# maikmerten/hmp3

Hardware: AMD Instinct MI355X
Metric: batched stereo 44.1kHz frames/sec (whole node), CBR-128 (higher is better)
Workload: dtype f32; 1 GPU; batch=1024 stereo 44.1kHz streams x 256 frames per step per GPU, CBR-128, long blocks only, int16 PCM resident in HBM; streams_per_gpu=1024, parallelism=streams sharded over 1 GPU(s), no collective

## Files before the change

hmp3_amd/csrc/hx_alloc.hip:

```cpp
#include "hx_dev.h"

#ifndef HX_LSF
#define HX_LSF 0
#endif
#ifndef HX_A1
#define HX_A1 0
#endif
#ifndef HX_SLIM
#define HX_SLIM 0
#endif
#if HX_SLIM && HX_A1
#error "the low-footprint layout is built for the second-generation allocator only"
#endif
#define HX_WAVES (HX_SLIM ? 3 : 2)
#define HX_PERSIST HX_SLIM
#define HX_RATE_SPEED (!HX_SLIM)
#define HX_OPAQUE_LANE HX_SLIM
#define HX_SEEK_FORCEINLINE HX_SLIM
#define HX_LUCKY_K (HX_SLIM ? 6 : 12)
#define GMIN_OFFSET 70
#define PART23 4021
#define NB 22

struct AllocPrm {
    unsigned char head[4];
    int remainder, divisor, main_framebytes, sf_bit_max, AveTargetBits;
    int ms_flag, hf_flag, vbr_flag;
    int ivbr_min, ivbr_max, vbr_main_framebytes[16], vbr_pool_target;
    int fbmin, fbmax;
    int initialMNR, test1;
    int nsf[2], nsf2[2], nsf3[2], nbmax[2], nbmax2[2], nbmax3[2];
    float rnBand_l[22];
    int nsfs, nbmax_s;
    struct { int npart; } psyS;
    int nchan, side_bytes;
    int is_flag, dual, npart_l;
    int oflags;
    int run_w;
};

static_assert(sizeof(HxGr) == 96, "the frame loop copies the four HxGr of a frame as 96 words");
struct alignas(16) Outbox {
    HxSegOut seg[2];
    HxGr gr[2][2];
    int scfsi[2], mdb, part;
    unsigned sidew[10];
    unsigned char head[4];
    HxFrameOut frm;
    HxSlot slot;
    int opos, frm_index, slot_index;
    int ring_p0;
    int has_frame;
};

#if HX_SLIM
typedef short ix_t;
typedef short sgs_t;
typedef signed char sfo_t;
typedef short btab_t;
#else
typedef int ix_t;
typedef int sgs_t;
typedef int sfo_t;
typedef int btab_t;
#endif

struct FrameState {
    int padcount; unsigned main_tot, main_sent, mf_tot;
    int main_bytes; unsigned side_p0, side_p1, tot_frames_out, tot_bytes_out; int ave_tot;
    int opos, slot_lo, slot_hi;
    int pad, byte_pool, byte_max, byte_min, bytesout, pk_first;
};

struct alignas(16) AllocLds {
    float xr[2][576];
    float x34[2][576];
    float term[2][576];
#if !HX_SLIM
    int ix[2][576];
    unsigned char signx[2][576];
    alignas(16) HxBandPrep band_next;
#else
    unsigned long long sgnbits[2][9];
    ix_t ixsink;
#endif
    unsigned char band_of_pair[288];
    unsigned short lane_run[64];
    unsigned char band_last[24];
    float look_ix43[256];
#if !HX_SLIM
    float look_gain[128], look_34igain[128];
    int mblog[256];
    float pow34_exp[256];
    int logsub[84];
#else
    float gain4[4], igain16[16];
    unsigned short mblog[256];
    short logsub[84];
#endif
    float pow34_a[16], pow34_b[16], quant_off[32];
    unsigned char huff_len[1408];
    unsigned char sband_of_line[192];
    btab_t nBand_s[16], startBand_s[16], logcbw_s[16];
    unsigned char quada_len[16];
    btab_t nBand[NB], startBand[24], logcbw[NB], taper[NB];
    int NTadjust[2][NB];
    union {
        struct {
            int snr[2][NB], Noise0[2][NB], Noise[2][NB], NT[2][NB];
            int gzero[2][NB], gmin[2][NB], gsf[2][NB], sf[2][NB], active[2][NB];
            int ixmax[2][NB], ix10xmax[2][NB], up[2][NB], lo[2][NB], geval[2][NB], maskmb[2][NB];
            float xsxx[2][NB], x34max[2][NB];
            float gig[2][NB];
            alignas(8) float2 gpair[2][NB];
            int lucky[HX_LUCKY_K][2][13];
            unsigned short llist[HX_LUCKY_K * 26 + 4];
        };
        struct {
            int a_pad[17][2][NB];
            float a_sig[2][NB], a_smask[2][NB], a_mask[2][NB], a_noise[2][NB];
            int a_lastGsf[2][NB];
        };
        struct {
            int s_snr[2][3][16], s_Noise0[2][3][16], s_Noise[2][3][16], s_NT[2][3][16];
            sgs_t s_gzero[2][3][16], s_gmin[2][3][16], s_gsf[2][3][16], s_sf[2][3][16], s_active[2][3][16];
            int s_ixmax[2][3][16], s_geval[3][16], s_tmpn[3][16], s_maskmb[2][3][16];
            float s_xsxx[2][3][16], s_x34max[2][3][16];
            int s_G[2][3], s_GG[2], s_subgain[2][3];
        };
    };
    int G[2], preemp[2], scale[2], huff_bits[2];
    int hs_table[2][4], hs_cbreg[2][3], hs_nbig[2], hs_nquads[2], hs_bits[2];
    int MNR, PoolFraction, call_count;
    int a_calls, a_bitadjust[2];
    float a_running, a_ave, a_alpha;
    int hf_quant, hf_quant_stereo[2], gsf_hf, gsf_hf_stereo[2];
    int sf_save[2][21];
    int scfsi[2];
    int nchan, block_type, maxBits, maxTargetBits, minTargetBits, PoolBits, TargetBits, deltaMNR, activeBands;
    int tmp[8];
    int tmpn[2][NB];
    unsigned int sidew[10];
    HxGr gr[2][2];
    sfo_t sfout[2][2][NB];
    sfo_t sfs[2][3][12];
    AllocPrm P;
    FrameState fs;
    int tabpk[32];
    unsigned long long candpk[19];
    unsigned short r_mf[32];
    int r_off[32];
#if !HX_SLIM
    float dump[64];
#endif
    Outbox ob[2];
    const double *pow43;
    int *big_counter;
    int nstrict;
#if !HX_SLIM
    int nlucky[3];
#endif
    int cur_s;
    alignas(16) int cmdw[4];
    alignas(4) unsigned char gflag[HX_SLIM ? 64 : 256];
#ifdef HX_PROFILE
    unsigned prof[HX_PROF_WORDS];
#endif
};

#if !HX_SLIM
static_assert(offsetof(AllocLds, ix) == offsetof(AllocLds, term) + sizeof(float) * 2 * 576 && sizeof(int) == sizeof(float),
              "big_lucky_noise's terms run on from the term buffer into the quantised lines: 2304 words in one piece");
#endif

#if HX_SLIM
#define IX(c) (reinterpret_cast<ix_t *>(&L.term[0][0]) + 576 * (c))
#define BAND_LANDING (reinterpret_cast<HxBandPrep *>(&L.term[1][0]))
#define LANE_SINK (reinterpret_cast<float *>(&L.lucky[0][0][0]) + LANE)
#define MBLOG(x) hx_mblog16(L.mblog, (x))
__device__ __forceinline__ float lk_gain(const float *g4, int g) { const int k = g - 8; return ldexpf(g4[k & 3], k >> 2); }
__device__ __forceinline__ float lk_igain(const float *ig16, int g) { const int k = g - 8; return ldexpf(ig16[k & 15], -3 * (k >> 4)); }
#define LK_GAIN(g) lk_gain(L.gain4, (g))
#define LK_IGAIN(g) lk_igain(L.igain16, (g))
#define LK_GAIN_RAW(g) L.gain4[((g) - 8) & 3]
#define LK_GAIN_FIN(raw, g) ldexpf((raw), ((g) - 8) >> 2)
#define LK_IGAIN_RAW(g) L.igain16[((g) - 8) & 15]
#define LK_IGAIN_FIN(raw, g) ldexpf((raw), -3 * (((g) - 8) >> 4))
#else
#define IX(c) (&L.ix[(c)][0])
#define BAND_LANDING (&L.band_next)
#define LANE_SINK (&L.dump[LANE])
#define MBLOG(x) hx_mblog(L.mblog, (x))
#define LK_GAIN(g) L.look_gain[(g)]
#define LK_IGAIN(g) L.look_34igain[(g)]
#define LK_GAIN_RAW(g) L.look_gain[(g)]
#define LK_GAIN_FIN(raw, g) (raw)
#define LK_IGAIN_RAW(g) L.look_34igain[(g)]
#define LK_IGAIN_FIN(raw, g) (raw)
#endif
#define BAND_OF_LINE(j) L.band_of_pair[(j) >> 1]

#ifdef HX_PROFILE
#define PROF(id, stmt) do { HX_WAVE_SYNC(); long long t0_ = clock64(); stmt; HX_WAVE_SYNC(); if (threadIdx.x == 0) L.prof[(id)] += (unsigned) (clock64() - t0_); } while (0)
#define PROF_T0() long long tp_ = clock64()
#define PROF_T1() tp_ = clock64()
#define PROF_CNT(id) do { if (threadIdx.x == 0) L.prof[(id)] += 1; } while (0)
#define PROF_ACC(id) do { HX_WAVE_SYNC(); if (threadIdx.x == 0) L.prof[(id)] += (unsigned) (clock64() - tp_); tp_ = clock64(); } while (0)
#define PROF_CLOCK , long long &tp_
#define PROF_PASS , tp_
#else
#define PROF(id, stmt) do { stmt; } while (0)
#define PROF_T0() do { } while (0)
#define PROF_T1() do { } while (0)
#define PROF_CNT(id) do { } while (0)
#define PROF_ACC(id) do { } while (0)
#define PROF_CLOCK
#define PROF_PASS
#endif
#define HX_COLD __attribute__((noinline, cold))
#define HX_HFN __attribute__((noinline))
#if HX_RATE_SPEED
#define HX_RATE __attribute__((noinline))
#else
#define HX_RATE HX_COLD
#endif
__device__ __forceinline__ int hx_lane_opaque()
{
    int l;
    asm volatile("v_mbcnt_lo_u32_b32 %0, -1, 0\n\tv_mbcnt_hi_u32_b32 %0, -1, %0" : "=v"(l));
    return l;
}
#if HX_OPAQUE_LANE
// ... 593 lines not shown
        if (!(s >= s0) || (GG - s) >= g0) mode = 2;
    }
    while (__any(mode == 1)) {
        PROF_CNT(HX_PROF_N_LUCKY);
        PROF_T0();
        int nc = 0;
        if (mode == 1) {
            const int sh = 1 + L.scale[ch];
            nc = min(K, min(((s - s0) >> sh) + 1, (g0 - GG + s + sdelta - 1) >> sh));
        }
        if (i < NB) { L.geval[ch][i] = (mode == 1) ? GG - s : -1; L.tmpn[ch][i] = nc; }
        unsigned short *list = L.llist;
        const int incl = hx_wave_scan(nc), total = __builtin_amdgcn_readlane(incl, 63);
#pragma unroll
        for (int c = 0; c < HX_LUCKY_K; c++) if (c < nc) list[incl - nc + c] = (c << 8) | (ch << 7) | i;
        HX_WAVE_SYNC();
        const int ncmax = hx_wave_max(nc);
#if !HX_SLIM
        npass++; reach = max(reach, ncmax);
#endif
        const bool bslow = mode == 1 && noise_band_needs_pow(LK_IGAIN(GG - s), L.x34max[ch][i]);
        PROF_ACC(HX_PROF_LUCKY_SETUP);
        const bool two = p->nchan == 2;
        const int big = __any(bslow) ? 1 : 0;
        if (two) { if (LANE == 0) L.cmdw[3] = big; HELPER_POST2(HCMD_LUCKY, nl, ncmax); }
        lucky_dispatch(L, nl, ncmax, tf, 0, big);
        if (two) HELPER_JOIN();
        else lucky_dispatch(L, nl, ncmax, tf, 1, big);
        HX_WAVE_SYNC();
        PROF_ACC(HX_PROF_LUCKY_TERMS);
        for (int u = LANE; u < total; u += 64) {
            const int e = list[u], c = e >> 8, cc = (e >> 7) & 1, b = e & 31;
            float sxx = band_sum(tf + c * 2 * nl + cc * nl + L.startBand[b], L.nBand[b], 0.0f);
            L.lucky[c][cc][b] = MBLOG(1.0e-12f + sxx) - L.logcbw[b];
        }
        HX_WAVE_SYNC();
        PROF_ACC(HX_PROF_LUCKY_SUMS);
        {
            int best = 0;
            bool hit = false;
#pragma unroll
            for (int h = 0; h < HX_LUCKY_K; h += 6) {
                if (h == 0 || ncmax > h) {
                    int nz[6];
#pragma unroll
                    for (int c = 0; c < 6; c++) nz[c] = L.lucky[h + c][ch][min(i, 12)];
#pragma unroll
                    for (int c = 0; c < 6; c++)
                        if (h + c < nc && nz[c] <= nt) { best = nz[c]; smin = s - (h + c) * sdelta; hit = true; }
                }
            }
            if (hit) L.Noise[ch][i] = best;
            if (mode == 1) {
                s -= nc * sdelta;
                if (!(s >= s0) || (GG - s) >= g0) mode = 2;
            }
        }
        HX_WAVE_SYNC();
        PROF_ACC(HX_PROF_LUCKY_REPLAY);
    }
    if (mode == 2) {
        L.sf[ch][i] = smin;
        L.gsf[ch][i] = max(GG - smin, 0);
    }
#if !HX_SLIM
    if (reach * 2 * nl > 1152) {
        const int end = reach * 2 * nl - 1152;
        for (int j = p->nbmax[0] + LANE; j < min(end, 576); j += 64) IX(0)[j] = 0;
        for (int j = p->nbmax[1] + LANE; j < end - 576; j += 64) IX(1)[j] = 0;
    }
    if (npass && LANE == 0) { L.nlucky[0] += 1; L.nlucky[1] += npass; L.nlucky[2] += (reach > 6); }
#endif
    HX_WAVE_SYNC();
}

__device__ __forceinline__ void quant_lines(AllocLds &L, const AllocPrm *p, int opt, int c)
{
    HX_LANE_DECL;
    const int nl = p->nbmax[c];
#if HX_SLIM
    const int nfill = (opt & 2) ? nl : 576;
#endif
    const bool tab = (opt & 1) != 0;
    int q[9], b[9];
#pragma unroll
    for (int k = 0; k < 9; k++) b[k] = BAND_OF_LINE(LANE + 64 * k);
#pragma unroll
    for (int k = 0; k < 9; k++) {
        const int j = LANE + 64 * k;
        const float igain = L.gig[c][b[k]];
        const float t = igain * L.x34[c][j] + (tab ? (0.5f - 0.4375f) : (0.5f - 0.0946f));
        const float off = L.quant_off[max(min((int) t, 31), 0)];
        q[k] = (int) (t - (tab ? off : 0.0f));
    }
#pragma unroll
    for (int k = 0; k < 9; k++) {
        const int j = LANE + 64 * k;
#if HX_SLIM
        const int qq = (j < nl) ? q[k] : 0;
        *((j < nfill) ? &IX(c)[j] : &L.ixsink) = (ix_t) qq;
        if (qq > 0) atomicMax(&L.ixmax[c][b[k]], qq);
#else
        if (j < nl) {
            IX(c)[j] = q[k];
            if (q[k] > 0) atomicMax(&L.ixmax[c][b[k]], q[k]);
        }
#endif
    }
}

__device__ void do_quant(AllocLds &L, const AllocPrm *p, int opt)
{
    HX_LANE_DECL;
    const int ch = LANE >> 5, i = LANE & 31;
    if (i < NB) {
        L.ixmax[ch][i] = (i < p->nsf[ch]) ? 0 : L.ixmax[ch][i];
        L.gig[ch][i] = LK_IGAIN(L.gsf[ch][i] & 127);
    }
    HX_WAVE_SYNC();
    const bool two = p->nbmax[1] > 0;
    if (two) HELPER_POST(HCMD_QUANT, opt);
    quant_lines(L, p, opt, 0);
    if (two) HELPER_JOIN();
    HX_WAVE_SYNC();
}

struct Cand { int n, t0, t1, t2, t3, tmax; };

__device__ __forceinline__ Cand mk_cand(int n, int t0, int t1, int t2, int t3, int tmax)
{
    Cand c; c.n = n; c.t0 = t0; c.t1 = t1; c.t2 = t2; c.t3 = t3; c.tmax = tmax;
    return c;
}

__device__ __forceinline__ Cand candidates_chain(int rmax)
{
    if (rmax <= 0) return mk_cand(0, 0, 0, 0, 0, 0);
    if (rmax == 1) return mk_cand(2, 1, 3, 0, 0, 1);
    if (rmax == 2) return mk_cand(2, 2, 3, 0, 0, 2);
    if (rmax == 3) return mk_cand(2, 5, 6, 0, 0, 3);
    if (rmax <= 5) return mk_cand(4, 7, 8, 9, 12, 5);
    if (rmax <= 7) return mk_cand(4, 10, 11, 12, 15, 7);
    if (rmax <= 15) return mk_cand(2, 13, 15, 0, 0, 15);
    if (rmax == 16) return mk_cand(2, 16, 24, 0, 0, 16);
    if (rmax <= 18) return mk_cand(2, 17, 24, 0, 0, 18);
    if (rmax <= 22) return mk_cand(2, 18, 24, 0, 0, 22);
    if (rmax <= 30) return mk_cand(2, 19, 24, 0, 0, 30);
    if (rmax <= 46) return mk_cand(2, 25, 20, 0, 0, 46);
    if (rmax <= 78) return mk_cand(2, 20, 26, 0, 0, 78);
    if (rmax <= 142) return mk_cand(2, 27, 21, 0, 0, 142);
    if (rmax <= 270) return mk_cand(2, 21, 28, 0, 0, 270);
    if (rmax <= 526) return mk_cand(2, 29, 22, 0, 0, 526);
    if (rmax <= 1038) return mk_cand(2, 22, 30, 0, 0, 1038);
    if (rmax <= 2062) return mk_cand(2, 30, 23, 0, 0, 2062);
    return mk_cand(2, 31, 23, 0, 0, 8206);
}

__device__ __forceinline__ int cand_class(int rmax)
{
    if (rmax <= 3) return max(rmax, 0);
    if (rmax <= 15) return rmax <= 5 ? 4 : (rmax <= 7 ? 5 : 6);
    return min(7 + (31 - __clz(rmax - 15)), 18);
}
__device__ __forceinline__ int cand_class_rep(int c)
{
    return c <= 3 ? c : (c == 4 ? 4 : (c == 5 ? 6 : (c == 6 ? 8 : 15 + (1 << (c - 7)))));
}
__device__ __forceinline__ unsigned long long cand_pack(const Cand &c)
{
    return (unsigned long long) (c.n | (c.t0 << 3) | (c.t1 << 8) | (c.t2 << 13) | (c.t3 << 18)) | ((unsigned long long) c.tmax << 23);
}
__device__ __forceinline__ Cand candidates(const AllocLds &L, int rmax)
{
    const unsigned long long pk = L.candpk[cand_class(rmax)];
    const unsigned lo = (unsigned) pk;
    return mk_cand(lo & 7, (lo >> 3) & 31, (lo >> 8) & 31, (lo >> 13) & 31, (lo >> 18) & 31, (int) (pk >> 23));
}

__device__ __forceinline__ int tab_pack(const AllocLds &L, int t) { return L.tabpk[t]; }
__device__ __forceinline__ int pair_len_p(const AllocLds &L, int pk, int x, int y)
{
    const int off = pk & 0xFFF, dim = (pk >> 12) & 0xFF, lin = pk >> 20;
    const int cx = min(x, 15), cy = min(y, 15);
    int n = L.huff_len[off + cx * dim + cy];
    n += (x >= 15 ? lin : 0) + (y >= 15 ? lin : 0);
    return n + (x != 0) + (y != 0);
}

__device__ __forceinline__ int pair_len(const AllocLds &L, int t, int x, int y) { return pair_len_p(L, tab_pack(L, t), x, y); }

__device__ __forceinline__ void acc_pair(const AllocLds &L, const Cand &c, int x, int y, int &p01, int &p23)
{
    if (c.n == 0) return;
    p01 += pair_len(L, c.t0, x, y) | (pair_len(L, c.t1, x, y) << 16);
    if (c.n == 4) p23 += pair_len(L, c.t2, x, y) | (pair_len(L, c.t3, x, y) << 16);
}

__device__ __forceinline__ int pick_table(const Cand &c, int p01, int p23, int live, int *bits)
{
    const int b0 = p01 & 0xFFFF, b1 = (p01 >> 16) & 0xFFFF, b2 = p23 & 0xFFFF, b3 = (p23 >> 16) & 0xFFFF;
    int best = 0, t = c.t0;
    if (c.n != 0 && live) {
        if (b0 < b1) { best = b0; t = c.t0; } else { best = b1; t = c.t1; }
        if (c.n == 4) {
            if (b2 <= best) { best = b2; t = c.t2; }
            if (b3 <= best) { best = b3; t = c.t3; }
        }
    }
    *bits += best;
    return t;
}

__device__ __forceinline__ int region_max(const int *ixmax, int a, int b)
{
    int m = 0;
    for (int i = a; i < b; i++) if (m < ixmax[i]) m = ixmax[i];
    return m;
}

__device__ int count_bits_ch(AllocLds &L, const AllocPrm *p, int ch, int ncb)
{
    HX_LANE_DECL;
    const int *ixmax = L.ixmax[ch];
    const ix_t *ix = IX(ch);
    const int bt = L.block_type;
    PROF_T0();
    int cb0, cb1, cb2, cb3;
    const int my = (LANE < ncb) ? ixmax[LANE] : 0;
    const unsigned long long mk0 = __ballot(my > 0), mk1 = __ballot(my > 1);
    cb3 = mk0 ? 64 - __clzll((long long) mk0) : 0;
    cb2 = mk1 ? 64 - __clzll((long long) mk1) : 0;
    cb0 = cb1 = 0;
#define RMAX(a_, b_) hx_wave_max((LANE >= (a_) && LANE < (b_)) ? my : 0)
    if (bt == 0) { if (cb2 < 2) { cb2 = 2; if (cb3 < cb2) cb3 = cb2; } }
    else { cb0 = 8; cb2 = max(cb2, 8); cb3 = max(cb3, cb2); cb1 = cb0; }
    PROF_ACC(HX_PROF_CNT_BALLOTS);
    int lo2 = L.startBand[cb2 - 1], hi2 = L.startBand[cb2], lo3 = L.startBand[cb3 - 1], hi3 = L.startBand[cb3];
    int j2 = lo2, j3 = lo3;
    for (int j = lo2 + LANE; j < hi2; j += 64) if (ix[j] > 1) j2 = j;
    for (int j = lo3 + LANE; j < hi3; j += 64) if (ix[j] > 0) j3 = j;
    j2 = hx_wave_max(j2);
    j3 = hx_wave_max(j3);
    PROF_ACC(HX_PROF_CNT_J23);
    int nbig = (j2 + 2) & (~1);
    if (bt == 0) { if (nbig < L.startBand[2]) nbig = L.startBand[2]; }
    else { if (nbig < L.startBand[8]) nbig = L.startBand[8]; }
    int nquads = (j3 + 4 - nbig) >> 2;
    if (bt != 0) nquads = max(nquads, 0);
    Cand c0, c1, c2;
    if (bt == 0) {
        const int c = cb2;
        int r0 = (c < 6) ? 1 : (c < 9 ? 2 : (c < 12 ? 3 : (c < 15 ? 4 : (c < 18 ? 5 : (c < 21 ? 6 : 7)))));
        int r1 = (c < 5) ? 1 : (c < 8 ? 2 : (c < 10 ? 3 : (c == 10 ? 4 : (c < 15 ? 5 : (c < 17 ? 6 : (c < 20 ? 7 : 8))))));
        cb0 = r0;
        cb1 = r0 + r1;
        if (cb0 < 1) cb0 = 1;
        if (cb1 <= cb0) cb1 = cb0 + 1;
        if (cb1 > cb0 + 8) cb1 = cb0 + 8;
        c0 = candidates(L, RMAX(0, cb0));
        c1 = candidates(L, RMAX(cb0, cb1));
        c2 = candidates(L, RMAX(cb1, cb2));
        if (c2.tmax < c1.tmax) {
            const unsigned long long m = __ballot(my > c2.tmax && LANE > cb0 && LANE <= cb1 - 1);
            const int j = m ? 63 - __clzll((long long) m) : cb0;
            cb1 = j + 1;
        }
        if (c1.tmax < c0.tmax) {
            int n = cb1 - 8;
            if (n < 1) n = 1;
            if (cb0 - 1 > n) {
                const unsigned long long m = __ballot(my > c1.tmax && LANE > n && LANE <= cb0 - 1);
                const int j = m ? 63 - __clzll((long long) m) : n;
                cb0 = j + 1;
            }
        }
    } else {
        c0 = candidates(L, RMAX(0, cb0));
        c1 = candidates(L, 0);
        c2 = candidates(L, RMAX(cb0, cb2));
    }
#undef RMAX
    PROF_ACC(HX_PROF_CNT_REGIONS);
    const int n0 = L.startBand[cb0], n1 = L.startBand[cb1];
    int r0a = 0, r0b = 0, r1a = 0, r1b = 0, r2a = 0, r2b = 0;
    {
        const int pa0 = tab_pack(L, c0.t0), pb0 = tab_pack(L, c0.t1);
        const int pa1 = tab_pack(L, c1.t0), pb1 = tab_pack(L, c1.t1);
        const int pa2 = tab_pack(L, c2.t0), pb2 = tab_pack(L, c2.t1);
        const bool any4 = c0.n == 4 || c1.n == 4 || c2.n == 4;
        int2 xy[5];
#pragma unroll
#if HX_SLIM
        for (int k = 0; k < 5; k++) { const unsigned w = reinterpret_cast<const unsigned *>(ix)[min(LANE + 64 * k, 287)]; xy[k] = make_int2((int) (w & 0xFFFFu), (int) (w >> 16)); }
#else
        for (int k = 0; k < 5; k++) xy[k] = reinterpret_cast<const int2 *>(ix)[min(LANE + 64 * k, 287)];
#endif
        int acc[5];
#pragma unroll
        for (int k = 0; k < 5; k++) {
            const int j = 2 * (LANE + 64 * k);
            const int pa = (j < n0) ? pa0 : (j < n1 ? pa1 : pa2), pb = (j < n0) ? pb0 : (j < n1 ? pb1 : pb2);
            acc[k] = pair_len_p(L, pa, xy[k].x, xy[k].y) | (pair_len_p(L, pb, xy[k].x, xy[k].y) << 16);
        }
#pragma unroll
        for (int k = 0; k < 5; k++) {
            const int j = 2 * (LANE + 64 * k);
            const int rn = (j < n0) ? c0.n : (j < n1 ? c1.n : c2.n);
            const int v = (j < nbig && rn != 0) ? acc[k] : 0;
            r0a += (j < n0) ? v : 0;
            r1a += (j >= n0 && j < n1) ? v : 0;
            r2a += (j >= n1) ? v : 0;
        }
        if (any4) {
            const int qa0 = tab_pack(L, c0.t2), qb0 = tab_pack(L, c0.t3);
            const int qa1 = tab_pack(L, c1.t2), qb1 = tab_pack(L, c1.t3);
            const int qa2 = tab_pack(L, c2.t2), qb2 = tab_pack(L, c2.t3);
#pragma unroll
            for (int k = 0; k < 5; k++) {
                const int j = 2 * (LANE + 64 * k);
                const int pa = (j < n0) ? qa0 : (j < n1 ? qa1 : qa2), pb = (j < n0) ? qb0 : (j < n1 ? qb1 : qb2);
                acc[k] = pair_len_p(L, pa, xy[k].x, xy[k].y) | (pair_len_p(L, pb, xy[k].x, xy[k].y) << 16);
            }
#pragma unroll
            for (int k = 0; k < 5; k++) {
                const int j = 2 * (LANE + 64 * k);
                const int rn = (j < n0) ? c0.n : (j < n1 ? c1.n : c2.n);
                const int v = (j < nbig && rn == 4) ? acc[k] : 0;
                r0b += (j < n0) ? v : 0;
                r1b += (j >= n0 && j < n1) ? v : 0;
                r2b += (j >= n1) ? v : 0;
            }
        }
    }
    PROF_ACC(HX_PROF_CNT_PAIRS);
    int qa = 0, qb = 0;
    {
        int2 qv[3][2];
#pragma unroll
        for (int k = 0; k < 3; k++) {
            const int q = min(LANE + 64 * k, max(nquads - 1, 0));
#if HX_SLIM
            const uint2 w2 = *reinterpret_cast<const uint2 *>(ix + nbig + 4 * q);
            qv[k][0] = make_int2((int) (w2.x & 0xFFFFu), (int) (w2.x >> 16)); qv[k][1] = make_int2((int) (w2.y & 0xFFFFu), (int) (w2.y >> 16));
#else
            const int2 *v2 = reinterpret_cast<const int2 *>(ix + nbig + 4 * q);
            qv[k][0] = v2[0]; qv[k][1] = v2[1];
#endif
        }
#pragma unroll
        for (int k = 0; k < 3; k++) {
            const int v0 = qv[k][0].x, v1 = qv[k][0].y, v2 = qv[k][1].x, v3 = qv[k][1].y;
            const int pop = v0 + v1 + v2 + v3;
            const int la = L.quada_len[((v0 << 3) + (v1 << 2) + (v2 << 1) + v3) & 15] + pop;
            const bool ok = LANE + 64 * k < nquads;
            qa += ok ? la : 0;
            qb += ok ? 4 + pop : 0;
        }
    }
    PROF_ACC(HX_PROF_CNT_QUADS);
    r0a = hx_wave_sum(r0a); r2a = hx_wave_sum(r2a);
    r0b = hx_wave_sum(r0b); r2b = hx_wave_sum(r2b);
    r1a = hx_wave_sum(r1a); r1b = hx_wave_sum(r1b);
    int bits = 0;
    const int tab0 = pick_table(c0, r0a, r0b, n0 > 0, &bits);
    int tab1 = pick_table(c1, r1a, r1b, (n1 - n0 > 0) && bt == 0, &bits);
    const int tab2 = pick_table(c2, r2a, r2b, nbig - n1 > 0, &bits);
    if (bt != 0) tab1 = tab2;
    {
        const int q = hx_wave_sum(qa | (qb << 16));
        qa = q & 0xFFFF;
        qb = (q >> 16) & 0xFFFF;
    }
    int qidx = 0;
    if (nquads > 0) { if (qa < qb) { bits += qa; qidx = 0; } else { bits += qb; qidx = 1; } }
    if (LANE == 0) {
        L.hs_table[ch][0] = tab0; L.hs_table[ch][1] = tab1; L.hs_table[ch][2] = tab2; L.hs_table[ch][3] = qidx;
        L.hs_cbreg[ch][0] = cb0; L.hs_cbreg[ch][1] = cb1; L.hs_cbreg[ch][2] = cb2;
        L.hs_nbig[ch] = nbig; L.hs_nquads[ch] = nquads; L.hs_bits[ch] = bits;
        L.huff_bits[ch] = bits;
    }
    PROF_ACC(HX_PROF_CNT_REDUCE);
    return bits;
}

__device__ int count_bits(AllocLds &L, const AllocPrm *p, const int *ncb)
{
    HX_LANE_DECL;
    PROF_CNT(HX_PROF_N_COUNTS);
    const bool two = p->nchan == 2;
    if (two) HELPER_POST(HCMD_COUNT_BITS, ncb[1]);
    int bits = count_bits_ch(L, p, 0, ncb[0]);
    if (two) { HELPER_JOIN(); bits += L.hs_bits[1]; }
    HX_WAVE_SYNC();
    return bits;
}

__device__ int quant_count_bits(AllocLds &L, const AllocPrm *p, int opt, int zero21, const int *ncb)
{
    HX_LANE_DECL;
    const int ch = LANE >> 5, i = LANE & 31;
    if (i < NB) {
        L.ixmax[ch][i] = (i < p->nsf[ch]) ? 0 : L.ixmax[ch][i];
        L.gig[ch][i] = LK_IGAIN(L.gsf[ch][i] & 127);
    }
    HX_WAVE_SYNC();
    PROF_CNT(HX_PROF_N_COUNTS);
    const bool two = p->nchan == 2;
    PROF_T0();
    if (two) HELPER_POST2(HCMD_QUANT_COUNT, opt, ncb[1]);
    PROF_ACC(HX_PROF_QC_POST);
    quant_lines(L, p, opt, 0);
    HX_WAVE_SYNC();
    PROF_ACC(HX_PROF_QC_QUANT);
    if (zero21) { if (LANE == 0) L.ixmax[0][21] = 0; HX_WAVE_SYNC(); }
    int bits = count_bits_ch(L, p, 0, ncb[0]);
    PROF_T1();
    if (two) { HELPER_JOIN(); bits += L.hs_bits[1]; }
    HX_WAVE_SYNC();
    PROF_ACC(HX_PROF_QC_JOIN);
    return bits;
}

#include "hx_alloc2.inc"
#include "hx_alloc_short.inc"
#if HX_A1
#include "hx_alloc1.inc"
#endif
#include "hx_alloc3.inc"
```

hmp3_amd/csrc/hx_alloc3.inc:

```

#define COLD(field) (((const __attribute__((address_space(4))) AllocArgs *) __builtin_amdgcn_kernarg_segment_ptr())->field)
#define RFL(x) __builtin_amdgcn_readfirstlane(x)

__device__ __noinline__ void emit_packet(AllocLds &L, const AllocPrm *p, unsigned char *q, int *nbytes, int pad, int ms, int raw_bytes, int hdr, int lsf_igr)
{
    HX_LANE_DECL;
    if (LANE < 4) {
        unsigned char h = p->head[LANE];
        if (LANE == 2 && pad) h |= 2;
        if (LANE == 3) h = (unsigned char) ((h & 0xCF) | ((ms + ms + (HX_A1 ? p->is_flag : 0)) << 4));
        q[LANE] = h;
    }
    if (lsf_igr >= 0) pack_side_lsf(L, p, q + 4, lsf_igr, 0);
    else pack_side(L, p, q + 4, 0);
    if (LANE == 0) *nbytes = hdr + raw_bytes;
}

template <int LSF>
__device__ __forceinline__ int pack_sf_any(AllocLds &L, int pos, int igr, int ch, int bt, int use_scfsi, int not_null, int *sc, unsigned short *sfdst)
{
    HX_LANE_DECL;
    *sc = 0;
    int field = 0;
    if (LSF) {
// ... 199 lines not shown
    for (int k = 0; k < 9; k++) { a[k] = L.xr[0][LANE + 64 * k]; b[k] = L.xr[1][LANE + 64 * k]; }
#pragma unroll
    for (int k = 0; k < 9; k++) {
        const int j = LANE + 64 * k;
        L.x34[0][j] = (j < nl0) ? pow34(L, a[k]) : 0.0f;
        L.x34[1][j] = (j < nl1) ? pow34(L, b[k]) : 0.0f;
    }
}

template <int LSF>
__device__ __forceinline__ void helper_serve(const AllocArgs &a, AllocLds &L)
{
    for (;;) {
        HX_LANE_DECL;
        WG_BARRIER();
        const int4 order = *reinterpret_cast<const int4 *>(&L.cmdw[0]);
        const int cmd = order.x;
        if (cmd == HCMD_SEEK) seek_actual_ch(L, &L.P, 1);
        else if (cmd == HCMD_COUNT_BITS) count_bits_ch(L, &L.P, 1, order.y);
        else if (cmd == HCMD_LUCKY) lucky_dispatch(L, order.y, order.z, &L.term[0][0], 1, order.w);
        else if (cmd == HCMD_QUANT) quant_lines(L, &L.P, order.y, 1);
        else if (cmd == HCMD_QUANT_COUNT) { quant_lines(L, &L.P, order.y, 1); HX_WAVE_SYNC(); count_bits_ch(L, &L.P, 1, order.z); }
        else if (cmd == HCMD_ISF2) isf2_ch(L, &L.P, 1);
        else if (cmd == HCMD_FETCH) {
            const int s = L.cur_s;
            int nbt = 2, nms = 0;
            if (order.y >= 0) {
                granule_fetch(L, a, (long long) s * a.NG + order.y);
                nbt = a.bt[(long long) s * a.NG + order.y]; nms = a.msflag[(long long) s * a.NG + order.y];
            }
            const int gl = order.z, gf = (gl >= 0) ? gl - 1 : ((order.y < 0) ? order.w : -1);
            LinesRegs lr0 = {}, lr1 = {};
            OutRegs orr = {};
            const int two = L.P.nchan == 2;
            const int gbt = order.w & 255;
            if (gl >= 0) { lines_gather(L, (order.w >> 8) & 1, 0, gbt, lr0); if (two) lines_gather(L, (order.w >> 9) & 1, 1, gbt, lr1); }
            if (gf >= 0) outbox_gather(L, gf, orr);
            asm volatile("s_waitcnt vmcnt(0) lgkmcnt(0)" ::: "memory");
            const bool long_gr = !HX_A1 && nbt != 2;
            if (long_gr) {
                xr_to_coded(L, nms);
                if (!two) x34_from_coded(L, nms);
                asm volatile("s_waitcnt lgkmcnt(0)" ::: "memory");
            }
            WG_BARRIER();
            if (gl >= 0) {
                const long long unit = (long long) s * a.NG + gl;
                lines_store(a, unit, 0, gbt, lr0);
                if (two) lines_store(a, unit, 1, gbt, lr1);
            }
            if (gf >= 0) outbox_store<LSF>(L, a, s, gf, orr);
            if (long_gr && two) { x34_from_coded(L, nms); asm volatile("s_waitcnt lgkmcnt(0)" ::: "memory"); }
            continue;
        }
        else if (cmd == HCMD_EXIT) return;
        WG_BARRIER();
    }
}

__device__ __forceinline__ void stage_stream(const AllocArgs &a, AllocLds &L, const HxStream *ss, const HxParams *gp, const HxGlobalTabs *gt)
{
    HX_LANE_DECL;
#if HX_SLIM
    for (int i = LANE; i < 256; i += 64) { L.look_ix43[i] = gp->look_ix43[i]; L.mblog[i] = (unsigned short) (gt->mblog[i] + 38227); }
    if (LANE < 4) L.gain4[LANE] = gp->look_gain[8 + LANE];
    if (LANE < 16) L.igain16[LANE] = gp->look_34igain[8 + LANE];
    if (LANE < 18) L.sgnbits[LANE / 9][LANE % 9] = 0;
#else
    for (int i = LANE; i < 256; i += 64) { L.look_ix43[i] = gp->look_ix43[i]; L.mblog[i] = gt->mblog[i]; L.pow34_exp[i] = gt->pow34_exp[i]; }
    for (int i = LANE; i < 128; i += 64) { L.look_gain[i] = gp->look_gain[i]; L.look_34igain[i] = gp->look_34igain[i]; }
#endif
    for (int i = LANE; i < 1408; i += 64) L.huff_len[i] = gt->huff_len[i];
    for (int i = LANE; i < 288; i += 64) L.band_of_pair[i] = gp->band_of_line[2 * i];
    L.lane_run[LANE] = gp->lane_run[LANE];
    if (LANE < 24) L.band_last[LANE] = gp->band_last_lane[LANE];
    for (int i = LANE; i < 192; i += 64) L.sband_of_line[i] = gp->sband_of_line[i];
    if (LANE < 16) {
        L.nBand_s[LANE] = (LANE < 13) ? gp->nBand_s[LANE] : 0;
        L.startBand_s[LANE] = (LANE < 14) ? gp->startBand_s[LANE] : 192;
        L.logcbw_s[LANE] = gp->look_log_cbwmb_s[LANE];
    }
    for (int i = LANE; i < 84; i += 64) L.logsub[i] = (HX_SLIM ? (short) gt->logsub[i] : gt->logsub[i]);
    if (LANE < 32) L.quant_off[LANE] = gt->quant_off[LANE];
    if (LANE < 32) {
        const int dim = (LANE >= 16) ? 16 : gt->huff_dim[LANE], lin = (LANE >= 16) ? gt->huff_lin[LANE] : 0;
        L.tabpk[LANE] = gt->huff_off[LANE] | (dim << 12) | (lin << 20);
    }
    if (LANE < 19) L.candpk[LANE] = cand_pack(candidates_chain(cand_class_rep(LANE)));
    if (LANE < 16) {
        L.pow34_a[LANE] = gt->pow34_a[LANE]; L.pow34_b[LANE] = gt->pow34_b[LANE];
        L.quada_len[LANE] = gt->quada_len[LANE];
    }
    if (LANE < 24) L.startBand[LANE] = gp->startBand_l[LANE];
    if (LANE < NB) { L.nBand[LANE] = gp->nBand_l[LANE]; L.logcbw[LANE] = gp->look_log_cbwmb[LANE]; L.taper[LANE] = gp->taperNT[LANE]; }
#if !HX_SLIM
    for (int i = LANE; i < 2 * 576; i += 64) { IX(0)[i] = 0; (&L.signx[0][0])[i] = 0; }
#endif
    if (LANE < 44) {
        int c = LANE / 22, b = LANE % 22;
        L.NTadjust[c][b] = ss->NTadjust[c][b];
        L.ixmax[c][b] = 0; L.sf[c][b] = 0; L.active[c][b] = 0; L.gsf[c][b] = 0; L.gzero[c][b] = 0; L.gmin[c][b] = 0;
        L.x34max[c][b] = 0.0f; L.Noise[c][b] = 0; L.Noise0[c][b] = 0; L.NT[c][b] = 0; L.geval[c][b] = -1;
        L.up[c][b] = 0; L.lo[c][b] = 0;
    }
    if (LANE < 42) L.sf_save[LANE / 21][LANE % 21] = ss->sf_save[LANE / 21][LANE % 21];
    if (LANE == 0) { L.pow43 = gt->pow43; L.big_counter = COLD(done_counter) + HX_CNT_BIG_SWEEPS; L.nstrict = 0; }
#if !HX_SLIM
    if (LANE < 3) L.nlucky[LANE] = 0;
#endif
    if (LANE < 4) L.P.head[LANE] = gp->head[LANE];
    if (LANE < 16) L.P.vbr_main_framebytes[LANE] = gp->vbr_main_framebytes[LANE];
    if (LANE < 22) L.P.rnBand_l[LANE] = gp->rnBand_l[LANE];
    if (LANE < 2) {
        const bool on = LANE < gp->nchan;
        L.P.nsf[LANE] = on ? gp->nsf[LANE] : 0; L.P.nsf2[LANE] = on ? gp->nsf2[LANE] : 0; L.P.nsf3[LANE] = on ? gp->nsf3[LANE] : 0;
        L.P.nbmax[LANE] = on ? gp->nbmax[LANE] : 0; L.P.nbmax2[LANE] = on ? gp->nbmax2[LANE] : 0; L.P.nbmax3[LANE] = on ? gp->nbmax3[LANE] : 0;
    }
    if (LANE == 0) {
        L.P.remainder = gp->remainder; L.P.divisor = gp->divisor; L.P.main_framebytes = gp->main_framebytes;
        L.P.sf_bit_max = gp->sf_bit_max; L.P.AveTargetBits = gp->AveTargetBits;
        L.P.ms_flag = gp->ms_flag; L.P.hf_flag = gp->hf_flag; L.P.vbr_flag = gp->vbr_flag;
        L.P.ivbr_min = gp->ivbr_min; L.P.ivbr_max = gp->ivbr_max; L.P.vbr_pool_target = gp->vbr_pool_target;
        L.P.fbmin = gp->vbr_main_framebytes[gp->ivbr_min & 15]; L.P.fbmax = gp->vbr_main_framebytes[gp->ivbr_max & 15];
        L.P.initialMNR = gp->initialMNR; L.P.test1 = gp->test1;
        L.P.nsfs = gp->nsfs; L.P.nbmax_s = gp->nbmax_s; L.P.psyS.npart = gp->psyS.npart;
        L.P.nchan = gp->nchan; L.P.side_bytes = gp->side_bytes;
        L.P.is_flag = gp->is_flag; L.P.dual = gp->alloc1 && gp->h_mode == 2; L.P.npart_l = gp->psyL.npart;
        L.P.oflags = (a.packet ? 1 : 0) | (a.dbg ? 2 : 0) | (a.frame_stats ? 4 : 0) | (a.strict_sums ? 8 : 0);
        L.P.run_w = gp->run_w;
    }
#if HX_A1
    for (int i = LANE; i < 256; i += 64) {
        (&L.term[0][0])[i] = gp->a1_f_ix[i]; (&L.term[0][0])[256 + i] = gp->a1_f_ixmax[i];
        (&L.term[0][0])[512 + i] = gp->a1_f_big_ix[i]; (&L.term[0][0])[768 + i] = gp->a1_f_big_ixmax[i];
    }
    if (LANE < 42) L.gsf[LANE / 21][LANE % 21] = ss->a1_gsf[LANE / 21][LANE % 21];
    if (LANE == 0) {
        L.a_calls = ss->a1_call_count; L.a_bitadjust[0] = ss->a1_bitadjust[0]; L.a_bitadjust[1] = ss->a1_bitadjust[1];
        L.a_running = ss->a1_running_a; L.a_ave = ss->a1_ave_alpha; L.a_alpha = ss->a1_alpha;
    }
#endif
    if (LANE == 0) {
        L.MNR = ss->MNR; L.PoolFraction = ss->PoolFraction; L.call_count = ss->call_count;
        L.hf_quant = 0; L.hf_quant_stereo[0] = L.hf_quant_stereo[1] = 0; L.gsf_hf = -1;
        L.gsf_hf_stereo[0] = L.gsf_hf_stereo[1] = -1;
        L.scfsi[0] = L.scfsi[1] = 0;
        for (int g = 0; g < 2; g++) for (int c = 0; c < 2; c++) {
            HxGr z = {};
            L.gr[g][c] = z;
            for (int k = 0; k < 3; k++) L.gr[g][c].subblock_gain[k] = ss->gr_subblock_gain[g][c][k];
        }
    }
#ifdef HX_PROFILE
    L.prof[LANE] = 0;
    if (LANE == 0) L.prof[HX_PROF_TOTAL] = (unsigned) clock64();
#endif
    HX_WAVE_SYNC();
}

template <int LSF>
__device__ __forceinline__ void slots_init(const AllocArgs &a, AllocLds &L, int s, const HxStream *ss, const HxParams *gp)
{
    HX_LANE_DECL;
    const int F = a.NG / 2;
    if (LANE == 0) {
        FrameState &fs = L.fs;
        fs.padcount = ss->padcount;
        fs.main_tot = ss->main_tot; fs.main_sent = ss->main_sent; fs.mf_tot = ss->mf_tot;
        fs.main_bytes = ss->main_bytes;
        fs.side_p0 = ss->side_p0; fs.side_p1 = ss->side_p1;
        fs.tot_frames_out = ss->tot_frames_out; fs.tot_bytes_out = ss->tot_bytes_out;
// ... 480 lines not shown
```

Baseline: 18.02 million frames/s.

## Vectorize quantization and bit counting over line pairs with precomputed candidate tables

Quantization now processes lines in pairs, loading float2 x34 values and storing packed int2 or 16-bit pairs to cut LDS instruction count and atomics per line. Bit counting precomputes per-candidate Huffman table packs in LDS, reads startBand values through lane reads instead of LDS, merges the j2/j3 scans into one loop, and derives the middle region sum from a total sum so one wave reduction is dropped. Clipping, escape and sign terms are hoisted out of the per-table lookup, and the quad count is moved earlier in the non-slim path. In exchange the code grows more complex, adds more LDS for the candidate tables, and raises register pressure.

```diff
diff --git a/hmp3_amd/csrc/hx_alloc.hip b/hmp3_amd/csrc/hx_alloc.hip
--- a/hmp3_amd/csrc/hx_alloc.hip
+++ b/hmp3_amd/csrc/hx_alloc.hip
@@ -82,7 +82,7 @@
     alignas(16) HxBandPrep band_next;
 #else
     unsigned long long sgnbits[2][9];
-    ix_t ixsink;
+    alignas(4) ix_t ixsink[2];
 #endif
     unsigned char band_of_pair[288];
     unsigned short lane_run[64];
@@ -148,6 +148,9 @@
     FrameState fs;
     int tabpk[32];
     unsigned long long candpk[19];
+#if !HX_SLIM
+    alignas(16) int candtab[19][4];
+#endif
     unsigned short r_mf[32];
     int r_off[32];
 #if !HX_SLIM
@@ -907,28 +910,33 @@
     const int nfill = (opt & 2) ? nl : 576;
 #endif
     const bool tab = (opt & 1) != 0;
-    int q[9], b[9];
-#pragma unroll
-    for (int k = 0; k < 9; k++) b[k] = BAND_OF_LINE(LANE + 64 * k);
-#pragma unroll
-    for (int k = 0; k < 9; k++) {
-        const int j = LANE + 64 * k;
+    int q0[5], q1[5], b[5];
+#pragma unroll
+    for (int k = 0; k < 5; k++) b[k] = L.band_of_pair[min(LANE + 64 * k, 287)];
+#pragma unroll
+    for (int k = 0; k < 5; k++) {
         const float igain = L.gig[c][b[k]];
-        const float t = igain * L.x34[c][j] + (tab ? (0.5f - 0.4375f) : (0.5f - 0.0946f));
-        const float off = L.quant_off[max(min((int) t, 31), 0)];
-        q[k] = (int) (t - (tab ? off : 0.0f));
-    }
-#pragma unroll
-    for (int k = 0; k < 9; k++) {
-        const int j = LANE + 64 * k;
+        const float2 x = reinterpret_cast<const float2 *>(&L.x34[c][0])[min(LANE + 64 * k, 287)];
+        const float t0 = igain * x.x + (tab ? (0.5f - 0.4375f) : (0.5f - 0.0946f));
+        const float t1 = igain * x.y + (tab ? (0.5f - 0.4375f) : (0.5f - 0.0946f));
+        const float off0 = L.quant_off[max(min((int) t0, 31), 0)];
+        const float off1 = L.quant_off[max(min((int) t1, 31), 0)];
+        q0[k] = (int) (t0 - (tab ? off0 : 0.0f));
+        q1[k] = (int) (t1 - (tab ? off1 : 0.0f));
+    }
+#pragma unroll
+    for (int k = 0; k < 5; k++) {
+        const int i = LANE + 64 * k, j = 2 * i;
 #if HX_SLIM
-        const int qq = (j < nl) ? q[k] : 0;
-        *((j < nfill) ? &IX(c)[j] : &L.ixsink) = (ix_t) qq;
-        if (qq > 0) atomicMax(&L.ixmax[c][b[k]], qq);
+        const int a0 = (j < nl) ? q0[k] : 0, a1 = (j < nl) ? q1[k] : 0;
+        *((j < nfill) ? reinterpret_cast<unsigned *>(IX(c)) + i : reinterpret_cast<unsigned *>(&L.ixsink[0])) = ((unsigned) a0 & 0xFFFFu) | ((unsigned) a1 << 16);
+        const int m = max(a0, a1);
+        if (m > 0) atomicMax(&L.ixmax[c][b[k]], m);
 #else
         if (j < nl) {
-            IX(c)[j] = q[k];
-            if (q[k] > 0) atomicMax(&L.ixmax[c][b[k]], q[k]);
+            reinterpret_cast<int2 *>(IX(c))[i] = make_int2(q0[k], q1[k]);
+            const int m = max(q0[k], q1[k]);
+            if (m > 0) atomicMax(&L.ixmax[c][b[k]], m);
         }
 #endif
     }
@@ -950,11 +958,12 @@
     HX_WAVE_SYNC();
 }
 
-struct Cand { int n, t0, t1, t2, t3, tmax; };
+struct Cand { int n, t0, t1, t2, t3, tmax; int pk0, pk1, pk2, pk3; };
 
 __device__ __forceinline__ Cand mk_cand(int n, int t0, int t1, int t2, int t3, int tmax)
 {
     Cand c; c.n = n; c.t0 = t0; c.t1 = t1; c.t2 = t2; c.t3 = t3; c.tmax = tmax;
+    c.pk0 = c.pk1 = c.pk2 = c.pk3 = 0;
     return c;
 }
 
@@ -983,9 +992,8 @@
 
 __device__ __forceinline__ int cand_class(int rmax)
 {
-    if (rmax <= 3) return max(rmax, 0);
-    if (rmax <= 15) return rmax <= 5 ? 4 : (rmax <= 7 ? 5 : 6);
-    return min(7 + (31 - __clz(rmax - 15)), 18);
+    const int lo = max(rmax, 0), mid = rmax <= 5 ? 4 : (rmax <= 7 ? 5 : 6), hi = min(7 + (31 - __clz(max(rmax - 15, 1))), 18);
+    return rmax <= 3 ? lo : (rmax <= 15 ? mid : hi);
 }
 __device__ __forceinline__ int cand_class_rep(int c)
 {
@@ -995,14 +1003,34 @@
 {
     return (unsigned long long) (c.n | (c.t0 << 3) | (c.t1 << 8) | (c.t2 << 13) | (c.t3 << 18)) | ((unsigned long long) c.tmax << 23);
 }
+__device__ __forceinline__ int tab_pack(const AllocLds &L, int t) { return L.tabpk[t]; }
+template <bool UNIFORM = false>
 __device__ __forceinline__ Cand candidates(const AllocLds &L, int rmax)
 {
-    const unsigned long long pk = L.candpk[cand_class(rmax)];
-    const unsigned lo = (unsigned) pk;
-    return mk_cand(lo & 7, (lo >> 3) & 31, (lo >> 8) & 31, (lo >> 13) & 31, (lo >> 18) & 31, (int) (pk >> 23));
-}
-
-__device__ __forceinline__ int tab_pack(const AllocLds &L, int t) { return L.tabpk[t]; }
+    const int cls = cand_class(rmax);
+    const unsigned long long pk = L.candpk[cls];
+#if !HX_SLIM
+    int4 tp = *reinterpret_cast<const int4 *>(&L.candtab[cls][0]);
+#endif
+    unsigned lo = (unsigned) pk, hi = (unsigned) (pk >> 32);
+    if (UNIFORM) {
+        lo = __builtin_amdgcn_readfirstlane(lo); hi = __builtin_amdgcn_readfirstlane(hi);
+#if !HX_SLIM
+        tp.x = __builtin_amdgcn_readfirstlane(tp.x); tp.y = __builtin_amdgcn_readfirstlane(tp.y);
+        tp.z = __builtin_amdgcn_readfirstlane(tp.z); tp.w = __builtin_amdgcn_readfirstlane(tp.w);
+#endif
+    }
+    Cand c = mk_cand(lo & 7, (lo >> 3) & 31, (lo >> 8) & 31, (lo >> 13) & 31, (lo >> 18) & 31, (int) ((lo >> 23) | (hi << 9)));
+#if !HX_SLIM
+    c.pk0 = tp.x; c.pk1 = tp.y; c.pk2 = tp.z; c.pk3 = tp.w;
+#endif
+    return c;
+}
+#if HX_SLIM
+#define CAND_PK(c, i) tab_pack(L, (c).t##i)
+#else
+#define CAND_PK(c, i) ((c).pk##i)
+#endif
 __device__ __forceinline__ int pair_len_p(const AllocLds &L, int pk, int x, int y)
 {
     const int off = pk & 0xFFF, dim = (pk >> 12) & 0xFF, lin = pk >> 20;
@@ -1010,6 +1038,12 @@
     int n = L.huff_len[off + cx * dim + cy];
     n += (x >= 15 ? lin : 0) + (y >= 15 ? lin : 0);
     return n + (x != 0) + (y != 0);
+}
+
+__device__ __forceinline__ int pair_len_s(const AllocLds &L, int pk, int cx, int cy, int nsign, int nesc)
+{
+    const int off = pk & 0xFFF, dim = (pk >> 12) & 0xFF, lin = pk >> 20;
+    return L.huff_len[off + cx * dim + cy] + nesc * lin + nsign;
 }
 
 __device__ __forceinline__ int pair_len(const AllocLds &L, int t, int x, int y) { return pair_len_p(L, tab_pack(L, t), x, y); }
@@ -1043,15 +1077,55 @@
     return m;
 }
 
-__device__ int count_bits_ch(AllocLds &L, const AllocPrm *p, int ch, int ncb)
+__device__ __forceinline__ int hx_lane_val(int v, int lane) { return __builtin_amdgcn_readlane(v, __builtin_amdgcn_readfirstlane(lane)); }
+
+__device__ __forceinline__ int pair_of_lane(int lane, int k) { return min(lane + 64 * k, 287); }
+__device__ __forceinline__ void load_pairs(const ix_t *ix, int lane, int2 (&xy)[5])
+{
+#pragma unroll
+#if HX_SLIM
+    for (int k = 0; k < 5; k++) { const unsigned w = reinterpret_cast<const unsigned *>(ix)[pair_of_lane(lane, k)]; xy[k] = make_int2((int) (w & 0xFFFFu), (int) (w >> 16)); }
+#else
+    for (int k = 0; k < 5; k++) xy[k] = reinterpret_cast<const int2 *>(ix)[pair_of_lane(lane, k)];
+#endif
+}
+
+__device__ __forceinline__ void count_quads(const AllocLds &L, const ix_t *ix, int nbig, int nquads, int &qa, int &qb)
+{
+    HX_LANE_DECL;
+    int2 qv[3][2];
+#pragma unroll
+    for (int k = 0; k < 3; k++) {
+        const int q = min(LANE + 64 * k, max(nquads - 1, 0));
+#if HX_SLIM
+        const uint2 w2 = *reinterpret_cast<const uint2 *>(ix + nbig + 4 * q);
+        qv[k][0] = make_int2((int) (w2.x & 0xFFFFu), (int) (w2.x >> 16)); qv[k][1] = make_int2((int) (w2.y & 0xFFFFu), (int) (w2.y >> 16));
+#else
+        const int2 *v2 = reinterpret_cast<const int2 *>(ix + nbig + 4 * q);
+        qv[k][0] = v2[0]; qv[k][1] = v2[1];
+#endif
+    }
+#pragma unroll
+    for (int k = 0; k < 3; k++) {
+        const int v0 = qv[k][0].x, v1 = qv[k][0].y, v2 = qv[k][1].x, v3 = qv[k][1].y;
+        const int pop = v0 + v1 + v2 + v3;
+        const int la = L.quada_len[((v0 << 3) + (v1 << 2) + (v2 << 1) + v3) & 15] + pop;
+        const bool ok = LANE + 64 * k < nquads;
+        qa += ok ? la : 0;
+        qb += ok ? 4 + pop : 0;
+    }
+}
+
+__device__ __forceinline__ int count_bits_pairs(AllocLds &L, const AllocPrm *p, int ch, int ncb, const int2 (&xy)[5])
 {
     HX_LANE_DECL;
     const int *ixmax = L.ixmax[ch];
     const ix_t *ix = IX(ch);
-    const int bt = L.block_type;
+    const int my = (LANE < ncb) ? ixmax[LANE] : 0;
+    const int sb = L.startBand[min(LANE, 23)];
+    const int bt = __builtin_amdgcn_readfirstlane(L.block_type);
     PROF_T0();
     int cb0, cb1, cb2, cb3;
-    const int my = (LANE < ncb) ? ixmax[LANE] : 0;
     const unsigned long long mk0 = __ballot(my > 0), mk1 = __ballot(my > 1);
     cb3 = mk0 ? 64 - __clzll((long long) mk0) : 0;
     cb2 = mk1 ? 64 - __clzll((long long) mk1) : 0;
@@ -1060,19 +1134,27 @@
     if (bt == 0) { if (cb2 < 2) { cb2 = 2; if (cb3 < cb2) cb3 = cb2; } }
     else { cb0 = 8; cb2 = max(cb2, 8); cb3 = max(cb3, cb2); cb1 = cb0; }
     PROF_ACC(HX_PROF_CNT_BALLOTS);
-    int lo2 = L.startBand[cb2 - 1], hi2 = L.startBand[cb2], lo3 = L.startBand[cb3 - 1], hi3 = L.startBand[cb3];
+    const int lo2 = hx_lane_val(sb, cb2 - 1), hi2 = hx_lane_val(sb, cb2), lo3 = hx_lane_val(sb, cb3 - 1), hi3 = hx_lane_val(sb, cb3);
     int j2 = lo2, j3 = lo3;
-    for (int j = lo2 + LANE; j < hi2; j += 64) if (ix[j] > 1) j2 = j;
-    for (int j = lo3 + LANE; j < hi3; j += 64) if (ix[j] > 0) j3 = j;
+#pragma nounroll
+    for (int o = 0, w = max(hi2 - lo2, hi3 - lo3); o < w; o += 64) {
+        const int a2 = lo2 + o + LANE, a3 = lo3 + o + LANE;
+        const int v2 = ix[min(a2, 575)], v3 = ix[min(a3, 575)];
+        if (a2 < hi2 && v2 > 1) j2 = a2;
+        if (a3 < hi3 && v3 > 0) j3 = a3;
+    }
     j2 = hx_wave_max(j2);
     j3 = hx_wave_max(j3);
     PROF_ACC(HX_PROF_CNT_J23);
     int nbig = (j2 + 2) & (~1);
-    if (bt == 0) { if (nbig < L.startBand[2]) nbig = L.startBand[2]; }
-    else { if (nbig < L.startBand[8]) nbig = L.startBand[8]; }
+    nbig = max(nbig, hx_lane_val(sb, bt == 0 ? 2 : 8));
     int nquads = (j3 + 4 - nbig) >> 2;
     if (bt != 0) nquads = max(nquads, 0);
-    Cand c0, c1, c2;
+    int qa = 0, qb = 0;
+#if !HX_SLIM
+    count_quads(L, ix, nbig, nquads, qa, qb);
+    PROF_ACC(HX_PROF_CNT_QUADS);
+#endif
     if (bt == 0) {
         const int c = cb2;
         int r0 = (c < 6) ? 1 : (c < 9 ? 2 : (c < 12 ? 3 : (c < 15 ? 4 : (c < 18 ? 5 : (c < 21 ? 6 : 7)))));
@@ -1082,9 +1164,9 @@
         if (cb0 < 1) cb0 = 1;
         if (cb1 <= cb0) cb1 = cb0 + 1;
         if (cb1 > cb0 + 8) cb1 = cb0 + 8;
-        c0 = candidates(L, RMAX(0, cb0));
-        c1 = candidates(L, RMAX(cb0, cb1));
-        c2 = candidates(L, RMAX(cb1, cb2));
+    }
+    const Cand c0 = candidates<true>(L, RMAX(0, cb0)), c1 = candidates<true>(L, RMAX(cb0, cb1)), c2 = candidates<true>(L, RMAX(cb1, cb2));
+    if (bt == 0) {
         if (c2.tmax < c1.tmax) {
             const unsigned long long m = __ballot(my > c2.tmax && LANE > cb0 && LANE <= cb1 - 1);
             const int j = m ? 63 - __clzll((long long) m) : cb0;
@@ -1099,93 +1181,68 @@
                 cb0 = j + 1;
             }
         }
-    } else {
-        c0 = candidates(L, RMAX(0, cb0));
-        c1 = candidates(L, 0);
-        c2 = candidates(L, RMAX(cb0, cb2));
     }
 #undef RMAX
     PROF_ACC(HX_PROF_CNT_REGIONS);
-    const int n0 = L.startBand[cb0], n1 = L.startBand[cb1];
-    int r0a = 0, r0b = 0, r1a = 0, r1b = 0, r2a = 0, r2b = 0;
+    const int n0 = hx_lane_val(sb, cb0), n1 = hx_lane_val(sb, cb1);
+    int tta = 0, ttb = 0, r0a = 0, r0b = 0, r2a = 0, r2b = 0;
     {
-        const int pa0 = tab_pack(L, c0.t0), pb0 = tab_pack(L, c0.t1);
-        const int pa1 = tab_pack(L, c1.t0), pb1 = tab_pack(L, c1.t1);
-        const int pa2 = tab_pack(L, c2.t0), pb2 = tab_pack(L, c2.t1);
+        const int pa0 = CAND_PK(c0, 0), pb0 = CAND_PK(c0, 1);
+        const int pa1 = CAND_PK(c1, 0), pb1 = CAND_PK(c1, 1);
+        const int pa2 = CAND_PK(c2, 0), pb2 = CAND_PK(c2, 1);
         const bool any4 = c0.n == 4 || c1.n == 4 || c2.n == 4;
-        int2 xy[5];
-#pragma unroll
-#if HX_SLIM
-        for (int k = 0; k < 5; k++) { const unsigned w = reinterpret_cast<const unsigned *>(ix)[min(LANE + 64 * k, 287)]; xy[k] = make_int2((int) (w & 0xFFFFu), (int) (w >> 16)); }
-#else
-        for (int k = 0; k < 5; k++) xy[k] = reinterpret_cast<const int2 *>(ix)[min(LANE + 64 * k, 287)];
-#endif
-        int acc[5];
+        int acc[5], cx[5], cy[5], nsign[5], nesc[5];
+#pragma unroll
+        for (int k = 0; k < 5; k++) {
+            const int x = xy[k].x, y = xy[k].y;
+            cx[k] = min(x, 15); cy[k] = min(y, 15);
+            nsign[k] = (x != 0) + (y != 0);
+            nesc[k] = (x >= 15) + (y >= 15);
+        }
 #pragma unroll
         for (int k = 0; k < 5; k++) {
             const int j = 2 * (LANE + 64 * k);
             const int pa = (j < n0) ? pa0 : (j < n1 ? pa1 : pa2), pb = (j < n0) ? pb0 : (j < n1 ? pb1 : pb2);
-            acc[k] = pair_len_p(L, pa, xy[k].x, xy[k].y) | (pair_len_p(L, pb, xy[k].x, xy[k].y) << 16);
+            acc[k] = pair_len_s(L, pa, cx[k], cy[k], nsign[k], nesc[k]) | (pair_len_s(L, pb, cx[k], cy[k], nsign[k], nesc[k]) << 16);
         }
 #pragma unroll
         for (int k = 0; k < 5; k++) {
             const int j = 2 * (LANE + 64 * k);
             const int rn = (j < n0) ? c0.n : (j < n1 ? c1.n : c2.n);
             const int v = (j < nbig && rn != 0) ? acc[k] : 0;
+            tta += v;
             r0a += (j < n0) ? v : 0;
-            r1a += (j >= n0 && j < n1) ? v : 0;
             r2a += (j >= n1) ? v : 0;
         }
         if (any4) {
-            const int qa0 = tab_pack(L, c0.t2), qb0 = tab_pack(L, c0.t3);
-            const int qa1 = tab_pack(L, c1.t2), qb1 = tab_pack(L, c1.t3);
-            const int qa2 = tab_pack(L, c2.t2), qb2 = tab_pack(L, c2.t3);
+            const int qa0 = CAND_PK(c0, 2), qb0 = CAND_PK(c0, 3);
+            const int qa1 = CAND_PK(c1, 2), qb1 = CAND_PK(c1, 3);
+            const int qa2 = CAND_PK(c2, 2), qb2 = CAND_PK(c2, 3);
 #pragma unroll
             for (int k = 0; k < 5; k++) {
                 const int j = 2 * (LANE + 64 * k);
                 const int pa = (j < n0) ? qa0 : (j < n1 ? qa1 : qa2), pb = (j < n0) ? qb0 : (j < n1 ? qb1 : qb2);
-                acc[k] = pair_len_p(L, pa, xy[k].x, xy[k].y) | (pair_len_p(L, pb, xy[k].x, xy[k].y) << 16);
+                acc[k] = pair_len_s(L, pa, cx[k], cy[k], nsign[k], nesc[k]) | (pair_len_s(L, pb, cx[k], cy[k], nsign[k], nesc[k]) << 16);
             }
 #pragma unroll
             for (int k = 0; k < 5; k++) {
                 const int j = 2 * (LANE + 64 * k);
                 const int rn = (j < n0) ? c0.n : (j < n1 ? c1.n : c2.n);
                 const int v = (j < nbig && rn == 4) ? acc[k] : 0;
+                ttb += v;
                 r0b += (j < n0) ? v : 0;
-                r1b += (j >= n0 && j < n1) ? v : 0;
                 r2b += (j >= n1) ? v : 0;
             }
         }
     }
     PROF_ACC(HX_PROF_CNT_PAIRS);
-    int qa = 0, qb = 0;
-    {
-        int2 qv[3][2];
-#pragma unroll
-        for (int k = 0; k < 3; k++) {
-            const int q = min(LANE + 64 * k, max(nquads - 1, 0));
 #if HX_SLIM
-            const uint2 w2 = *reinterpret_cast<const uint2 *>(ix + nbig + 4 * q);
-            qv[k][0] = make_int2((int) (w2.x & 0xFFFFu), (int) (w2.x >> 16)); qv[k][1] = make_int2((int) (w2.y & 0xFFFFu), (int) (w2.y >> 16));
-#else
-            const int2 *v2 = reinterpret_cast<const int2 *>(ix + nbig + 4 * q);
-            qv[k][0] = v2[0]; qv[k][1] = v2[1];
-#endif
-        }
-#pragma unroll
-        for (int k = 0; k < 3; k++) {
-            const int v0 = qv[k][0].x, v1 = qv[k][0].y, v2 = qv[k][1].x, v3 = qv[k][1].y;
-            const int pop = v0 + v1 + v2 + v3;
-            const int la = L.quada_len[((v0 << 3) + (v1 << 2) + (v2 << 1) + v3) & 15] + pop;
-            const bool ok = LANE + 64 * k < nquads;
-            qa += ok ? la : 0;
-            qb += ok ? 4 + pop : 0;
-        }
-    }
+    count_quads(L, ix, nbig, nquads, qa, qb);
     PROF_ACC(HX_PROF_CNT_QUADS);
+#endif
     r0a = hx_wave_sum(r0a); r2a = hx_wave_sum(r2a);
     r0b = hx_wave_sum(r0b); r2b = hx_wave_sum(r2b);
-    r1a = hx_wave_sum(r1a); r1b = hx_wave_sum(r1b);
+    const int r1a = hx_wave_sum(tta) - r0a - r2a, r1b = hx_wave_sum(ttb) - r0b - r2b;
     int bits = 0;
     const int tab0 = pick_table(c0, r0a, r0b, n0 > 0, &bits);
     int tab1 = pick_table(c1, r1a, r1b, (n1 - n0 > 0) && bt == 0, &bits);
@@ -1208,6 +1265,14 @@
     return bits;
 }
 
+__device__ int count_bits_ch(AllocLds &L, const AllocPrm *p, int ch, int ncb)
+{
+    HX_LANE_DECL;
+    int2 xy[5];
+    load_pairs(IX(ch), LANE, xy);
+    return count_bits_pairs(L, p, ch, ncb, xy);
+}
+
 __device__ int count_bits(AllocLds &L, const AllocPrm *p, const int *ncb)
 {
     HX_LANE_DECL;
diff --git a/hmp3_amd/csrc/hx_alloc3.inc b/hmp3_amd/csrc/hx_alloc3.inc
--- a/hmp3_amd/csrc/hx_alloc3.inc
+++ b/hmp3_amd/csrc/hx_alloc3.inc
@@ -305,11 +305,18 @@
     }
     for (int i = LANE; i < 84; i += 64) L.logsub[i] = (HX_SLIM ? (short) gt->logsub[i] : gt->logsub[i]);
     if (LANE < 32) L.quant_off[LANE] = gt->quant_off[LANE];
-    if (LANE < 32) {
-        const int dim = (LANE >= 16) ? 16 : gt->huff_dim[LANE], lin = (LANE >= 16) ? gt->huff_lin[LANE] : 0;
-        L.tabpk[LANE] = gt->huff_off[LANE] | (dim << 12) | (lin << 20);
-    }
-    if (LANE < 19) L.candpk[LANE] = cand_pack(candidates_chain(cand_class_rep(LANE)));
+    const auto tabpk_of = [gt](int t) {
+        const int dim = (t >= 16) ? 16 : gt->huff_dim[t], lin = (t >= 16) ? gt->huff_lin[t] : 0;
+        return gt->huff_off[t] | (dim << 12) | (lin << 20);
+    };
+    if (LANE < 32) L.tabpk[LANE] = tabpk_of(LANE);
+    if (LANE < 19) {
+        const Cand c = candidates_chain(cand_class_rep(LANE));
+        L.candpk[LANE] = cand_pack(c);
+#if !HX_SLIM
+        L.candtab[LANE][0] = tabpk_of(c.t0); L.candtab[LANE][1] = tabpk_of(c.t1); L.candtab[LANE][2] = tabpk_of(c.t2); L.candtab[LANE][3] = tabpk_of(c.t3);
+#endif
+    }
     if (LANE < 16) {
         L.pow34_a[LANE] = gt->pow34_a[LANE]; L.pow34_b[LANE] = gt->pow34_b[LANE];
         L.quada_len[LANE] = gt->quada_len[LANE];
```

After: 18.18 million frames/s (median of 6 runs). Within noise of the previous version (+0.9%).
